# ArtyZe/yolo_quantization

Measured on AMD Instinct MI355X. Metric: images/sec yolov3-tiny INT8 416x416, higher is better.
Workload: dtype u8 x s8 -> int32 (f64 or exact-integer requant, bit-identical)

## Files before the change

yolo_quantization_amd/csrc/conv_rows.hip:

```cpp
#include "kargs.h"
#include <type_traits>

#if defined(MI355_ABLATE) && !defined(ROWS_TU_KS1)
#define DBG(bit) ((a.debug & (bit)) != 0)
#define TS_PHASES 6
#define TS_BLOCKS 4096
__device__ long long g_rows_ts[TS_PHASES][TS_BLOCKS];
#define TS(k)                                                                                   \
    do {                                                                                        \
        if (threadIdx.x == 0 && blockIdx.x < TS_BLOCKS) g_rows_ts[k][blockIdx.x] = wall_clock64(); \
    } while (0)
extern "C" int mi355_debug_read_ts(long long *host)
{
    return hipMemcpyFromSymbol(host, HIP_SYMBOL(g_rows_ts), sizeof(long long) * TS_PHASES * TS_BLOCKS) == hipSuccess ? 0 : -5;
}
#define WP_PHASES 5
__device__ long long g_rows_wp[TS_BLOCKS][8][WP_PHASES];
#define WP_DECL long long wp_acc[WP_PHASES] = {0, 0, 0, 0, 0}; long long wp_t = 0
#define WP_START()                                                   \
    do {                                                             \
        if (DBG(256)) { wp_t = __builtin_readcyclecounter(); }       \
    } while (0)
#define WP_MARK(k)                                                   \
    do {                                                             \
        if (DBG(256)) {                                              \
            asm volatile("s_waitcnt lgkmcnt(0)" ::: "memory");       \
            const long long wp_n = __builtin_readcyclecounter();     \
            wp_acc[k] += wp_n - wp_t;                                \
            wp_t = wp_n;                                             \
        }                                                            \
    } while (0)
#define WP_FLUSH()                                                                                   \
    do {                                                                                             \
        if (DBG(256) && lane == 0 && blockIdx.x < TS_BLOCKS && wave < 8)                             \
            for (int k = 0; k < WP_PHASES; ++k) g_rows_wp[blockIdx.x][wave][k] = wp_acc[k];          \
    } while (0)
extern "C" int mi355_debug_read_wp(long long *host)
{
    return hipMemcpyFromSymbol(host, HIP_SYMBOL(g_rows_wp), sizeof(long long) * TS_BLOCKS * 8 * WP_PHASES) == hipSuccess ? 0 : -5;
}
#else
#define DBG(bit) (false)
#define TS(k) do { } while (0)
#define WP_DECL do { } while (0)
#define WP_START() do { } while (0)
#define WP_MARK(k) do { } while (0)
#define WP_FLUSH() do { } while (0)
#endif

#define DMA16(gsrc, ldst)                                                                               \
    __builtin_amdgcn_global_load_lds((const __attribute__((address_space(1))) void *)(gsrc),           \
                                     (__attribute__((address_space(3))) void *)(ldst), 16, 0, 0)

template <int KS, int BN> constexpr int ra_stages() { return KS == 3 ? (BN <= 192 ? 4 : 6) : (BN <= 128 ? 4 : 3); }
template <int KS, int BN> constexpr int rb_stages() { return KS == 3 ? 2 : ra_stages<KS, BN>(); }
constexpr int rows_nb_slots(int BN, int RS, int NW, int KS)
{
    const int wmin = RS * 3 / 4, halo = KS == 3 ? 1 : 0;
    const int rows = (BN - 2 + wmin) / wmin + 1 + (BN - 2 + wmin * wmin) / (wmin * wmin) + 2 * halo;
    return (rows * (RS / 16) + NW - 1) / NW;
}

__device__ __forceinline__ void row_of_pixel(int n, int H, int W, FastDiv fd_hw, FastDiv fd_w, int &grow, int &x)
{
    const int hw = H * W;
    const int b = fd_div(n, fd_hw);
    const int r = n - b * hw;
    const int y = fd_div(r, fd_w);
    x = r - y * W;
    grow = b * (H + 1) + y + 1;
}

template <int BM, int BN, int WMW, int WNW, int RS, int KS>
__global__ __launch_bounds__(64 * WMW * WNW, 2) void conv_rows_i8_kernel(const ConvArgs a)
{
    constexpr int NW = WMW * WNW, NT = 64 * NW;
    constexpr int TM = BM / WMW, TN = BN / WNW;
    constexpr int MS = TM / 32, NS = TN / 32;
    constexpr int ACH = BM / 16;
    constexpr int DW = (NW == 8 && KS == 3) ? 4 : NW;
    constexpr int APT = (ACH + DW - 1) / DW;
    constexpr int HALO = (KS == 3) ? 1 : 0;
    constexpr int PIECEB = RS * 16;
    constexpr int CPR = RS / 16;
    constexpr int OSTR = BM + 4;
    constexpr int RA_STAGES = ra_stages<KS, BN>();
    constexpr int RB_STAGES = rb_stages<KS, BN>();
    constexpr int NBS = rows_nb_slots(BN, RS, DW, KS);
    constexpr int SPS = (NBS + 3) / 4;
    static_assert(TM % 32 == 0 && TN % 32 == 0, "wave tile must be a multiple of the 32x32 MFMA tile");

    extern __shared__ __attribute__((aligned(16))) char smem[];
    char *ldsA = smem;
    char *ldsB = smem + RA_STAGES * BM * 64;
    const int rowb = a.rowb;
    const int bbytes = a.rows_cap * rowb;
    int *ldsS = reinterpret_cast<int *>(ldsB + RB_STAGES * bbytes);
    double *ldsPM = reinterpret_cast<double *>(smem + a.lds_param_off);
    int *ldsPI = reinterpret_cast<int *>(ldsPM + 3 * BM);
    float *ldsYL = reinterpret_cast<float *>(ldsPI + 2 * BM);

    const int tid = threadIdx.x;
    const int lane = tid & 63;
    const int wave = __builtin_amdgcn_readfirstlane(tid >> 6);
    const int wm = wave / WNW, wn = wave % WNW;
    const int kh = lane >> 5, lj = lane & 31;
    const int dwave = wave & (DW - 1);
    const bool issuer = wave < DW;
    TS(0);

    int logical;
    {
        const int nb = gridDim.x, id = blockIdx.x;
        const int q = nb >> 3, r = nb & 7, xcd = id & 7, idx = id >> 3;
        logical = (xcd < r ? xcd * (q + 1) : r * (q + 1) + (xcd - r) * q) + idx;
    }
    int mtile, ntile;
    {
        const int blk = fd_div(logical, a.fd_ntper);
        const int rem = logical - blk * (a.xcd_mb * a.ntiles_n);
        ntile = fd_div(rem, a.fd_mb);
        mtile = blk * a.xcd_mb + (rem - ntile * a.xcd_mb);
    }
    const int n0 = ntile * a.tile_q + min(ntile, a.tile_r);
    const int n_end = n0 + a.tile_q + (ntile < a.tile_r ? 1 : 0);
    const int W1 = a.W + 1, hw = a.H * a.W;

    int gr0, x0;
    row_of_pixel(n0, a.H, a.W, a.fd_hw, a.fd_w, gr0, x0);
    int gr1, x1;
    row_of_pixel(n_end - 1, a.H, a.W, a.fd_hw, a.fd_w, gr1, x1);
    const int grow_first = gr0 - HALO;
    const int nrows = gr1 - gr0 + 1 + 2 * HALO;
    const int ndma = nrows * CPR;

    int bbase[NS];
    int prow[NS], pcol[NS];
    bool nvalid[NS];
#pragma unroll
    for (int ns = 0; ns < NS; ++ns) {
        const int n = n0 + (ns * WNW + wn) * 32 + lj;
        nvalid[ns] = n < n_end;
        int gr, x;
        row_of_pixel(nvalid[ns] ? n : n_end - 1, a.H, a.W, a.fd_hw, a.fd_w, gr, x);
        prow[ns] = gr - grow_first - HALO;
        pcol[ns] = x + 1 - HALO;
        bbase[ns] = prow[ns] * rowb + pcol[ns] * 16 + kh * PIECEB;
    }
    int atab[MS];
#pragma unroll
    for (int ms = 0; ms < MS; ++ms) {
        const int row = wm * TM + ms * 32 + lj;
        atab[ms] = ((row >> 4) << 10) + ((row & 15) << 4) + kh * 256;
    }

    const unsigned lds0 = (unsigned)(size_t)(__attribute__((address_space(3))) char *)smem;
#define DMA_S(ldsdst_u32, sbase_ptr, voff_u32)                                                                   \
    asm volatile("s_mov_b32 m0, %0\n\ts_nop 0\n\tglobal_load_lds_dwordx4 %1, %2" ::"s"(ldsdst_u32), "v"(voff_u32), \
                 "s"(sbase_ptr)                                                                                  \
                 : "memory", "m0")
    constexpr int TAPS = KS * KS;
    const int rot = a.debug & 512 ? 0 : ntile - fd_div(ntile, a.fd_nch) * a.nchunks;
    const int kwrap = a.ksteps;
    int aleft = kwrap - rot * TAPS;
    const int8_t *aptr[APT];
    unsigned adst[APT];
#pragma unroll
    for (int i = 0; i < APT; ++i) {
        const int ch = min(dwave + i * DW, ACH - 1);
        aptr[i] = a.wp + ((size_t)(mtile * ACH + ch) * a.ksteps + (size_t)rot * TAPS) * 1024;
        adst[i] = lds0 + (ch << 10);
    }
    const unsigned lane16 = lane * 16;
// ... 210 lines not shown
                        for (int ms = 0; ms < MS; ++ms) rot[st][ms] = aaddr[(st + ROT) % R][ms];
#pragma unroll
                    for (int st = 0; st < R; ++st)
#pragma unroll
                        for (int ms = 0; ms < MS; ++ms) aaddr[st][ms] = rot[st][ms];
#pragma unroll
                    for (int yy = 0; yy < 3; ++yy)
#pragma unroll
                        for (int ns = 0; ns < NS; ++ns) baddr[yy][ns] += bdelta;
                }
                WP_MARK(0);
                if (t > 0 || chunk > 0) {
                    asm volatile("s_waitcnt vmcnt(%0)" ::"n"(YOUNG) : "memory");
                    WP_MARK(1);
                    if (!DBG(2)) __builtin_amdgcn_s_barrier();
                    WP_MARK(2);
                }
                half(fa[C0], fb[C0], fa[N0], fb[N0], aaddr[SN], baddr[TYN], integral_constant<int, TAPN>{},
                     integral_constant<int, 0>{}, integral_constant<bool, RD>{}, true_type{}, [&] {
                         if (!LAST && t < 4 && !DBG(1))
                             issueB_slots(chunk + 1, integral_constant<int, BLO>{}, integral_constant<int, BHI>{});
                         if (ISSUE_A && !DBG(1)) {
                             if constexpr (R == 6) {
                                 constexpr unsigned E = ((t + R - 1) % R) * (BM * 64), O = ((t + R - 1 + 3) % R) * (BM * 64);
                                 issueA_next(odd ? O : E);
                             } else {
                                 issueA_next((unsigned)((chunk + t + R - 1) & 3) * (BM * 64));
                             }
                         }
                     });
                WP_MARK(3);
                half(fa[C1], fb[C1], fa[N1], fb[N1], aaddr[SN], baddr[TYN], integral_constant<int, TAPN>{},
                     integral_constant<int, 1>{}, integral_constant<bool, RD>{}, integral_constant<bool, RD>{}, nohook);
                WP_MARK(4);
                if (t == 1 && !DBG(16)) {
                    asm volatile("s_waitcnt lgkmcnt(0)" ::: "memory");
                    cell_sums(Bt);
                    asm volatile("s_waitcnt lgkmcnt(0)" ::: "memory");
                    __builtin_amdgcn_sched_barrier(0);
                }
            };
            step(integral_constant<int, 0>{}); step(integral_constant<int, 1>{}); step(integral_constant<int, 2>{});
            step(integral_constant<int, 3>{}); step(integral_constant<int, 4>{}); step(integral_constant<int, 5>{});
            step(integral_constant<int, 6>{}); step(integral_constant<int, 7>{}); step(integral_constant<int, 8>{});
        };
        for (int chunk = 0; chunk + 1 < a.nchunks; ++chunk) chunk_body(false_type{}, chunk);
        chunk_body(true_type{}, a.nchunks - 1);
        asm volatile("s_waitcnt lgkmcnt(0)" ::: "memory");
        WP_FLUSH();
#undef LDS_READ128
    } else {
        TS(2);
        constexpr int R1 = RA_STAGES;
        constexpr int G = NBS + APT;
        static_assert(RB_STAGES == R1 && (R1 == 3 || R1 == 4), "1x1 loop: common ring depth");
        for (int g0 = 0; g0 < a.ksteps; g0 += R1) {
#pragma unroll
            for (int u = 0; u < R1; ++u) {
                const int g = g0 + u;
                if (g < a.ksteps) {
                    const int young = min(R1 - 2, a.ksteps - 1 - g);
                    if (young == R1 - 2) asm volatile("s_waitcnt vmcnt(%0)" ::"n"((R1 - 2) * G) : "memory");
                    else if (young == 1) asm volatile("s_waitcnt vmcnt(%0)" ::"n"(G) : "memory");
                    else asm volatile("s_waitcnt vmcnt(0)" ::: "memory");
                    __builtin_amdgcn_s_barrier();
                    if (g + R1 - 1 < a.ksteps) {
                        issueB(g + R1 - 1);
                        issueA_next(((u + R1 - 1) % R1) * (BM * 64));
                    }
                    const char *Bt = ldsB + u * bbytes;
                    compute(ldsA + u * (BM * 64), Bt, 0);
                    __builtin_amdgcn_sched_barrier(0);
                }
            }
        }
    }

    TS(3);
    if (DBG(32)) {
        if (acc[0][0][0] == 0x7fffffff && a.y) a.y[tid] = 1;
        return;
    }
    __syncthreads();
    int sx[NS];
#pragma unroll
    for (int ns = 0; ns < NS; ++ns) {
        int t = 0;
        if (KS == 1) {
            t = sxr[ns] + __shfl_xor(sxr[ns], 32);
        } else {
            const int c0 = prow[ns] * RS + pcol[ns];
#pragma unroll
            for (int dy = 0; dy < KS; ++dy)
#pragma unroll
                for (int dx = 0; dx < KS; ++dx) t += ldsS[c0 + dy * RS + dx];
        }
        sx[ns] = t;
    }
    __syncthreads();
    char *otile = smem;
    int *celltab = reinterpret_cast<int *>(smem + BN * OSTR);
    const int m0 = mtile * BM;

    int pb_[NS], rem[NS], nl_[NS];
#pragma unroll
    for (int ns = 0; ns < NS; ++ns) {
        const int nl = (ns * WNW + wn) * 32 + lj;
        nl_[ns] = nl;
        const int nn = nvalid[ns] ? n0 + nl : 0;
        const int b = fd_div(nn, a.fd_hw);
        const int rem0 = nn - b * hw;
        const int y = fd_div(rem0, a.fd_w), xx = rem0 - y * a.W;
        pb_[ns] = b;
        rem[ns] = rem0;
        if (wm == 0 && kh == 0) {
            const int up = a.up;
            celltab[nl] = !nvalid[ns] ? -1
                          : up == 1   ? a.out_lead + (b * (a.H + 1) + (y + 1)) * W1 + xx
                                      : a.out_lead + (b * (up * a.H + 1) + (up * y + 1)) * (up * a.W + 1) + up * xx;
        }
    }
    const bool fast = !a.acc_out && a.hdr->pow2 == 1;
    auto epi_fast = [&](auto act_c, auto sat_c) {
        constexpr int ACT = decltype(act_c)::value;
        constexpr bool SAT = decltype(sat_c)::value != 0;
#pragma unroll
        for (int ms = 0; ms < MS; ++ms) {
#pragma unroll
            for (int grp = 0; grp < 4; ++grp) {
                const int ocl = wm * TM + ms * 32 + 8 * grp + 4 * kh;
                const int4 dz4 = *reinterpret_cast<const int4 *>(ldsPI + ocl);
                const int dzv[4] = {dz4.x, dz4.y, dz4.z, dz4.w};
                int32_t accb[4][NS];
                double mp[4];
#pragma unroll
                for (int r = 0; r < 4; ++r) {
                    mp[r] = ldsPM[2 * BM + ocl + r];
#pragma unroll
                    for (int ns = 0; ns < NS; ++ns)
                        accb[r][ns] = acc[ms][ns][grp * 4 + r] + __mul24(dzv[r], sx[ns]);
                }
                int32_t v[4][NS];
                requant_values<ACT, SAT, NS>(accb, mp, a.zp_act, v);
#pragma unroll
                for (int ns = 0; ns < NS; ++ns)
                    *reinterpret_cast<uint32_t *>(otile + nl_[ns] * OSTR + ocl) = pack4_biased(v[0][ns], v[1][ns], v[2][ns], v[3][ns]);
                if (a.y_f32) {
#pragma unroll
                    for (int r = 0; r < 4; ++r) {
                        const int oc = m0 + ocl + r;
                        if (oc < a.n) {
                            const int e = a.yolo_out ? oc % a.yolo_per : 0;
#pragma unroll
                            for (int ns = 0; ns < NS; ++ns)
                                if (nvalid[ns]) {
                                    const int u8 = v[r][ns] & 0xFF;
                                    const float f = (float)(u8 - a.zp_act) * a.s_act;
                                    const size_t ridx = ((size_t)pb_[ns] * a.n + oc) * hw + rem[ns];
                                    a.y_f32[ridx] = f;
                                    if (a.yolo_out) a.yolo_out[ridx] = (e == 2 || e == 3) ? f : ldsYL[u8];
                                }
                        }
                    }
                }
            }
        }
    };
    using std::integral_constant;
    if (DBG(64)) {
    } else if (fast) {
#ifdef MI355_EPI_ONE
        epi_fast(integral_constant<int, MI355_ACT_LEAKY>{}, integral_constant<int, 0>{});
    }
    if (false) {
#endif
        const bool sat = a.store_mode == MI355_STORE_SATURATE;
        if (a.act == MI355_ACT_LEAKY) {
            if (sat) epi_fast(integral_constant<int, MI355_ACT_LEAKY>{}, integral_constant<int, 1>{});
            else epi_fast(integral_constant<int, MI355_ACT_LEAKY>{}, integral_constant<int, 0>{});
        } else if (a.act == MI355_ACT_RELU6) {
            if (sat) epi_fast(integral_constant<int, MI355_ACT_RELU6>{}, integral_constant<int, 1>{});
            else epi_fast(integral_constant<int, MI355_ACT_RELU6>{}, integral_constant<int, 0>{});
        } else {
            if (sat) epi_fast(integral_constant<int, MI355_ACT_LINEAR>{}, integral_constant<int, 1>{});
            else epi_fast(integral_constant<int, MI355_ACT_LINEAR>{}, integral_constant<int, 0>{});
        }
    }
#ifndef MI355_EPI_ONE
    else {
    #pragma unroll
        for (int ms = 0; ms < MS; ++ms) {
    #pragma unroll
            for (int grp = 0; grp < 4; ++grp) {
                const int ocl = wm * TM + ms * 32 + 8 * grp + 4 * kh;
                const int oc0 = m0 + ocl;
                if (oc0 >= a.n) {
    #pragma unroll
                    for (int ns = 0; ns < NS; ++ns) *reinterpret_cast<uint32_t *>(otile + nl_[ns] * OSTR + ocl) = 0x80808080u;
                    continue;
                }
                uint32_t packed[NS];
    #pragma unroll
                for (int ns = 0; ns < NS; ++ns) packed[ns] = 0;
    #pragma unroll
                for (int r = 0; r < 4; ++r) {
                    const int oc = oc0 + r;
                    const int dzv = ldsPI[ocl + r], biv = ldsPI[BM + ocl + r];
                    const double mv = ldsPM[ocl + r], sv = ldsPM[BM + ocl + r];
    #pragma unroll
                    for (int ns = 0; ns < NS; ++ns) {
                        const int32_t accv = acc[ms][ns][grp * 4 + r] - biv + dzv * sx[ns];
                        uint32_t u8 = 0;
                        if (oc < a.n) {
                            u8 = requant_u8(accv, biv, mv, sv, a.zp_act, a.act, a.store_mode);
                            if (nvalid[ns] && (a.acc_out || a.y_f32)) {
                                const size_t ridx = ((size_t)pb_[ns] * a.n + oc) * hw + rem[ns];
                                if (a.acc_out) a.acc_out[ridx] = accv;
                                if (a.y_f32) {
                                    const float f = (float)((int)u8 - a.zp_act) * a.s_act;
                                    a.y_f32[ridx] = f;
                                    if (a.yolo_out) {
                                        const int e = oc % a.yolo_per;
                                        a.yolo_out[ridx] = (e == 2 || e == 3) ? f : ldsYL[u8];
                                    }
                                }
                            }
                        }
                        packed[ns] |= (u8 ^ 0x80u) << (8 * r);
                    }
                }
    #pragma unroll
                for (int ns = 0; ns < NS; ++ns) *reinterpret_cast<uint32_t *>(otile + nl_[ns] * OSTR + ocl) = packed[ns];
            }
        }
    }
#endif
    __syncthreads();
    TS(4);
    if (a.y && !DBG(128)) {
        const int dwords = min(BM, a.out_w - m0) >> 2;
        if (a.up > 1) {
            const int total = BN * dwords, rowc = a.up * a.W + 1;
            for (int p = tid; p < total; p += NT) {
                const int pix = p / dwords, d = p - pix * dwords;
                const int cell = celltab[pix];
                if (cell >= 0) {
                    const uint32_t v = *reinterpret_cast<const uint32_t *>(otile + pix * OSTR + d * 4);
                    for (int uy = 0; uy < a.up; ++uy)
                        for (int ux = 0; ux < a.up; ++ux)
                            *reinterpret_cast<uint32_t *>(a.y + (size_t)(cell + uy * rowc + ux) * a.out_cs + m0 + d * 4) = v;
                }
            }
        } else if (dwords == BM / 4 && !(a.out_cs & 15) && !((size_t)a.y & 15)) {
#pragma unroll 2
            for (int p = tid; p < BN * (BM / 16); p += NT) {
                const int pix = p / (BM / 16), q = p % (BM / 16);
                const int cell = celltab[pix];
                if (cell >= 0) {
                    const uint32_t *sp = reinterpret_cast<const uint32_t *>(otile + pix * OSTR + q * 16);
                    const uint4 v = make_uint4(sp[0], sp[1], sp[2], sp[3]);
                    *reinterpret_cast<uint4 *>(a.y + (size_t)cell * a.out_cs + m0 + q * 16) = v;
                }
            }
        } else if (dwords == BM / 4) {
#pragma unroll 4
            for (int p = tid; p < BN * (BM / 4); p += NT) {
                const int pix = p / (BM / 4), d = p % (BM / 4);
                const int cell = celltab[pix];
                if (cell >= 0)
                    *reinterpret_cast<uint32_t *>(a.y + (size_t)cell * a.out_cs + m0 + d * 4) =
                        *reinterpret_cast<const uint32_t *>(otile + pix * OSTR + d * 4);
            }
        } else {
            const int total = BN * dwords;
            for (int p = tid; p < total; p += NT) {
                const int pix = p / dwords, d = p - pix * dwords;
                const int cell = celltab[pix];
                if (cell >= 0)
                    *reinterpret_cast<uint32_t *>(a.y + (size_t)cell * a.out_cs + m0 + d * 4) =
                        *reinterpret_cast<const uint32_t *>(otile + pix * OSTR + d * 4);
            }
        }
    }
    TS(5);
}

template <int BM, int BN, int WMW, int WNW, int RS, int KS>
static int rows_launch_cfg(ConvArgs &a, hipStream_t st)
{
    constexpr int NW = WMW * WNW, NT = 64 * NW;
    constexpr int DW = (NW == 8 && KS == 3) ? 4 : NW;
    constexpr int HALO = (KS == 3) ? 1 : 0;
    if (a.mpad % BM) return MI355_EINVAL;
    a.mtiles = a.mpad / BM;
    if (a.ntiles_n < (a.total_n + BN - 1) / BN) a.ntiles_n = (a.total_n + BN - 1) / BN;
    a.rows_cap = (BN - 2 + a.W) / a.W + 1 + (BN - 2 + a.H * a.W) / (a.H * a.W) + 2 * HALO;
    const int ndma = a.rows_cap * (RS / 16);
    if ((ndma + DW - 1) / DW > rows_nb_slots(BN, RS, DW, KS)) return MI355_EINVAL;
    if ((size_t)a.in_cells * (size_t)a.in_cs >= ((size_t)1 << 32)) return MI355_EINVAL;
    a.rowb = RS * 64 + 16 * (a.W & 15);
    a.fd_hw = fastdiv_make((uint32_t)(a.H * a.W)); a.fd_w = fastdiv_make((uint32_t)a.W);
    a.fd_ntn = fastdiv_make((uint32_t)a.ntiles_n); a.fd_nch = fastdiv_make((uint32_t)a.nchunks);
    a.tile_q = a.total_n / a.ntiles_n; a.tile_r = a.total_n % a.ntiles_n;
    size_t lds = (size_t)ra_stages<KS, BN>() * BM * 64 + (size_t)rb_stages<KS, BN>() * a.rows_cap * a.rowb + (size_t)a.rows_cap * RS * 4;
    const size_t lds_epi = (size_t)BN * (BM + 4) + (size_t)BN * 4;
    if (lds_epi > lds) lds = lds_epi;
    lds = (lds + 15) & ~(size_t)15;
    a.lds_param_off = (int)lds;
    lds += (size_t)BM * 32 + (a.yolo_out ? 1024 : 0);
    if (lds > 160 * 1024) return MI355_EINVAL;
    auto kern = conv_rows_i8_kernel<BM, BN, WMW, WNW, RS, KS>;
    static size_t lds_attr_dev[64] = {0};
    int dev_ix = 0;
    (void)hipGetDevice(&dev_ix);
    size_t &lds_attr = lds_attr_dev[dev_ix & 63];
    if (lds > 64 * 1024 && lds > lds_attr) {
        lds_attr = lds;
        if (hipFuncSetAttribute(reinterpret_cast<const void *>(kern), hipFuncAttributeMaxDynamicSharedMemorySize,
                                (int)lds) != hipSuccess)
            return MI355_EHIP;
    }
    a.xcd_mb = 1;
    if (!(a.debug & (1 << 24))) {
        const long nb = (long)a.ntiles_n * a.mtiles, per = (nb + 7) / 8;
        const double wslab = (double)BM * a.ksteps * 64, itile = (double)a.total_n / a.ntiles_n * a.cb * a.nchunks;
        double best = 0;
        for (int mb = 1; mb <= a.mtiles; ++mb) {
            if (a.mtiles % mb) continue;
            const long blk = (long)mb * a.ntiles_n;
            const long mt = std::min<long>(a.mtiles, mb * ((per + blk - 1) / blk)), nt = std::min<long>(a.ntiles_n, (per + mb - 1) / mb + (per % mb || blk % per || nb % 8 ? 1 : 0));
            const double bytes = mt * wslab + nt * itile;
            if (mb == 1 || bytes < best) { best = bytes; a.xcd_mb = mb; }
        }
    }
    a.fd_ntper = fastdiv_make((uint32_t)(a.xcd_mb * a.ntiles_n));
    a.fd_mb = fastdiv_make((uint32_t)a.xcd_mb);
    dim3 grid(a.ntiles_n * a.mtiles), block(NT);
    conv_launch_note(grid.x, NT, lds);
    hipLaunchKernelGGL(kern, grid, block, lds, st, a);
    return hipGetLastError() == hipSuccess ? MI355_OK : MI355_EHIP;
}

template <int RS, int KS>
static int rows_launch_tile(ConvArgs &a, hipStream_t st, int bm, int bn)
{
    if (bm == 128 && bn == 384) return rows_launch_cfg<128, 384, 2, 4, RS, KS>(a, st);
    if (bm == 128 && bn == 256) return rows_launch_cfg<128, 256, 2, 4, RS, KS>(a, st);
    if constexpr (KS == 3) {
        if (bm == 128 && bn == 192) return rows_launch_cfg<128, 192, 2, 2, RS, KS>(a, st);
    }
    if (bm == 128 && bn == 128) return rows_launch_cfg<128, 128, 2, 2, RS, KS>(a, st);
    if (bm == 64 && bn == 256) return rows_launch_cfg<64, 256, 1, 4, RS, KS>(a, st);
    if (bm == 64 && bn == 128) return rows_launch_cfg<64, 128, 1, 4, RS, KS>(a, st);
    if (bm == 32 && bn == 256) return rows_launch_cfg<32, 256, 1, 4, RS, KS>(a, st);
    if (bm == 32 && bn == 128) return rows_launch_cfg<32, 128, 1, 4, RS, KS>(a, st);
    return MI355_EINVAL;
}

// ... 30 lines not shown
```

yolo_quantization_amd/csrc/conv_rows16.hip:

```cpp
#include "kargs.h"
#include <type_traits>

#if defined(MI355_ABLATE)
#define DBG(bit) ((a.debug & (bit)) != 0)
__device__ long long g_rows16_ts[6][4096];
#define TS(k) do { if (threadIdx.x == 0 && blockIdx.x < 4096) g_rows16_ts[k][blockIdx.x] = wall_clock64(); } while (0)
extern "C" int mi355_debug_read_ts16(long long *host)
{
    return hipMemcpyFromSymbol(host, HIP_SYMBOL(g_rows16_ts), sizeof(long long) * 6 * 4096) == hipSuccess ? 0 : -5;
}
#else
#define DBG(bit) (false)
#define TS(k) do { } while (0)
#endif
#define WP_DECL do { } while (0)
#define WP_START() do { } while (0)
#define WP_MARK(k) do { } while (0)
#define WP_FLUSH() do { } while (0)

#define DMA16(gsrc, ldst)                                                                               \
    __builtin_amdgcn_global_load_lds((const __attribute__((address_space(1))) void *)(gsrc),           \
                                     (__attribute__((address_space(3))) void *)(ldst), 16, 0, 0)

template <int KS, int BN> constexpr int ra16_stages() { return KS == 3 ? (BN <= 192 ? 4 : 6) : (BN <= 128 ? 4 : 3); }
template <int KS, int BN> constexpr int rb16_stages() { return KS == 3 ? 2 : ra16_stages<KS, BN>(); }
constexpr int rows16_nb_slots(int BN, int RS, int NW, int KS)
{
    const int wmin = RS * 3 / 4, halo = KS == 3 ? 1 : 0;
    const int rows = (BN - 2 + wmin) / wmin + 1 + (BN - 2 + wmin * wmin) / (wmin * wmin) + 2 * halo;
    return (rows * (RS / 16) + NW - 1) / NW;
}

__device__ __forceinline__ void row16_of_pixel(int n, int H, int W, FastDiv fd_hw, FastDiv fd_w, int &grow, int &x)
{
    const int hw = H * W;
    const int b = fd_div(n, fd_hw);
    const int r = n - b * hw;
    const int y = fd_div(r, fd_w);
    x = r - y * W;
    grow = b * (H + 1) + y + 1;
}

template <int BM, int BN, int WMW, int WNW, int RS, int KS, int NBX = 0>
__global__ __launch_bounds__(64 * WMW * WNW, (BM / WMW > 64 ? 1 : 2)) void conv_rows16_i8_kernel(const ConvArgs a)
{
    constexpr int NW = WMW * WNW, NT = 64 * NW;
    constexpr int TM = BM / WMW, TN = BN / WNW;
    constexpr int MI = TM / 16, NI = TN / 16;
    constexpr int ACH = BM / 16;
    static_assert(KS == 3 && TN % 32 == 0, "3x3 only; pixels are dealt in 32-column sub-tiles (two 16-column tiles each)");
    constexpr int DW = (NW == 8 && KS == 3) ? 4 : NW;
    constexpr int APT = (ACH + DW - 1) / DW;
    constexpr int HALO = (KS == 3) ? 1 : 0;
    constexpr int PIECEB = RS * 16;
    constexpr int CPR = RS / 16;
    constexpr int OSTR = BM + 4;
    constexpr int RA_STAGES = ra16_stages<KS, BN>();
    constexpr int RB_STAGES = rb16_stages<KS, BN>();
    constexpr int NBS = rows16_nb_slots(BN, RS, DW, KS) + NBX;
    constexpr int SPS = (NBS + 3) / 4;
    static_assert(TM % 16 == 0 && TN % 32 == 0, "wave tile: 16-row tiles, 32-column sub-tiles");
    constexpr int CPT = (NBS * DW * 16 + NT - 1) / NT;
    static_assert(CPT * NT >= NBS * DW * 16 && CPT >= 1 && CPT <= 2, "a chunk's 4 CPT piece reads ride on its K-steps 0..7, one each");
    constexpr bool COUNTED = CPT == 1;
    constexpr auto cs_slot = [](int t) { return !COUNTED ? -1 : CPT == 2 ? (t >= 0 && t < 8 ? t : -1) : (t >= 0 && t < 8 && !(t & 1) ? t >> 1 : -1); };

    extern __shared__ __attribute__((aligned(16))) char smem[];
    char *ldsB = smem + RA_STAGES * BM * 64;
    const int rowb = a.rowb;
    const int bbytes = a.rows_cap * rowb;
    int *ldsS = reinterpret_cast<int *>(ldsB + RB_STAGES * bbytes);
    double *ldsPM = reinterpret_cast<double *>(smem + a.lds_param_off);
    int *ldsPI = reinterpret_cast<int *>(ldsPM + 3 * BM);
    float *ldsYL = reinterpret_cast<float *>(ldsPI + 2 * BM);

    const int tid = threadIdx.x;
    const int lane = tid & 63;
    const int wave = __builtin_amdgcn_readfirstlane(tid >> 6);
    const int wm = wave / WNW, wn = wave % WNW;
    const int kq = lane >> 4, lj = lane & 15;
    const int dwave = wave & (DW - 1);
    const bool issuer = wave < DW;
    TS(0);

    int logical;
    {
        const int nb = gridDim.x, id = blockIdx.x;
        const int q = nb >> 3, r = nb & 7, xcd = id & 7, idx = id >> 3;
        logical = (xcd < r ? xcd * (q + 1) : r * (q + 1) + (xcd - r) * q) + idx;
    }
    int mtile, ntile;
    {
        const int blk = fd_div(logical, a.fd_ntper);
        const int rem = logical - blk * (a.xcd_mb * a.ntiles_n);
        ntile = fd_div(rem, a.fd_mb);
        mtile = blk * a.xcd_mb + (rem - ntile * a.xcd_mb);
    }
    const int n0 = ntile * a.tile_q + min(ntile, a.tile_r);
    const int n_end = n0 + a.tile_q + (ntile < a.tile_r ? 1 : 0);
    const int W1 = a.W + 1, hw = a.H * a.W;

    int gr0, x0;
    row16_of_pixel(n0, a.H, a.W, a.fd_hw, a.fd_w, gr0, x0);
    int gr1, x1;
    row16_of_pixel(n_end - 1, a.H, a.W, a.fd_hw, a.fd_w, gr1, x1);
    const int grow_first = gr0 - HALO;
    const int nrows = gr1 - gr0 + 1 + 2 * HALO;
    const int ndma = nrows * CPR;

    constexpr int NS = NI;
    int bbase[NS];
#pragma unroll
    for (int ns = 0; ns < NS; ++ns) {
        const int n = n0 + ((ns >> 1) * WNW + wn) * 32 + (ns & 1) * 16 + lj;
        int gr, x;
        row16_of_pixel(n < n_end ? n : n_end - 1, a.H, a.W, a.fd_hw, a.fd_w, gr, x);
        const int prow = gr - grow_first - HALO;
        const int pcol = x + 1 - HALO;
        bbase[ns] = prow * rowb + pcol * 16 + kq * PIECEB;
    }
    const int atab0 = (wm * MI) * 1024 + lane * 16;

    const unsigned lds0 = (unsigned)(size_t)(__attribute__((address_space(3))) char *)smem;
#define DMA_S(ldsdst_u32, sbase_ptr, voff_u32)                                                                   \
    asm volatile("s_mov_b32 m0, %0\n\ts_nop 0\n\tglobal_load_lds_dwordx4 %1, %2" ::"s"(ldsdst_u32), "v"(voff_u32), \
                 "s"(sbase_ptr)                                                                                  \
                 : "memory", "m0")
    constexpr int TAPS = KS * KS;
    const int rot = a.debug & 512 ? 0 : ntile - fd_div(ntile, a.fd_nch) * a.nchunks;
    const int kwrap = a.ksteps;
    int aleft = kwrap - rot * TAPS;
    const int8_t *aptr[APT];
    unsigned adst[APT];
#pragma unroll
    for (int i = 0; i < APT; ++i) {
        const int ch = min(dwave + i * DW, ACH - 1);
        aptr[i] = a.wp + ((size_t)(mtile * ACH + ch) * a.ksteps + (size_t)rot * TAPS) * 1024;
        adst[i] = lds0 + (ch << 10);
    }
    const unsigned lane16 = lane * 16;
    auto issueA_next = [&](unsigned stage_off) {
        if (DW < NW && !issuer) return;
// ... 180 lines not shown
                if (t == 2 || t == 5) {
#pragma unroll
                    for (int ni = 0; ni < NI; ++ni) baddr[ni] += rowb;
                }
                if (t > 0 || chunk > 0) {
                    asm volatile("s_waitcnt vmcnt(%0)" ::"n"(YOUNG) : "memory");
                    __builtin_amdgcn_s_barrier();
                }
                auto dma = [&] {
                    __builtin_amdgcn_sched_barrier(0);
                    if (!LAST && t < 4) issueB_slots(chunk + 1, integral_constant<int, BLO>{}, integral_constant<int, BHI>{});
                    if (ISSUE_A) {
                        if constexpr (R == 6) {
                            constexpr unsigned E = ((t + R - 1) % R) * (BM * 64), O = ((t + R - 1 + 3) % R) * (BM * 64);
                            issueA_next(odd ? O : E);
                        } else if constexpr (R == 5) {
                            issueA_next(sst[t == 8 ? (t + R - 1 - 9) % R : (t + R - 1) % R]);
                        } else {
                            issueA_next((unsigned)((chunk + t + R - 1) & 3) * (BM * 64));
                        }
                    }
                    __builtin_amdgcn_sched_barrier(0);
                };
                asm volatile("s_waitcnt lgkmcnt(2)" ::: "memory");
                __builtin_amdgcn_sched_barrier(0);
#pragma unroll
                for (int ni = 0; ni < NI - 2; ++ni) {
#pragma unroll
                    for (int mi = 0; mi < MI; ++mi) {
                        acc[mi][ni] = __builtin_amdgcn_mfma_i32_16x16x64_i8(fa[mi], fb[ni], acc[mi][ni], 0, 0, 0);
                        if (ni == 0 && mi == 0) dma();
                    }
                    __builtin_amdgcn_sched_barrier(0);
                    if (RD) LDS_READ128(fb[ni], baddr[ni], TAPN);
                    __builtin_amdgcn_sched_barrier(0);
                    if (ni == 0) cell_piece();
                }
                if (RD) asm volatile("s_waitcnt lgkmcnt(%0)" ::"n"(NI - 2 + (NI > 2 && CJ >= 0 ? 1 : 0)) : "memory");
                else asm volatile("s_waitcnt lgkmcnt(0)" ::: "memory");
                __builtin_amdgcn_sched_barrier(0);
#pragma unroll
                for (int mi = 0; mi < MI; ++mi) {
                    acc[mi][NI - 2] = __builtin_amdgcn_mfma_i32_16x16x64_i8(fa[mi], fb[NI - 2], acc[mi][NI - 2], 0, 0, 0);
                    if (NI == 2 && mi == 0) dma();
                    acc[mi][NI - 1] = __builtin_amdgcn_mfma_i32_16x16x64_i8(fa[mi], fb[NI - 1], acc[mi][NI - 1], 0, 0, 0);
                    __builtin_amdgcn_sched_barrier(0);
                    if (RD) LDS_READ128(fa[mi], aaddr[SN], mi * 1024);
                    __builtin_amdgcn_sched_barrier(0);
                    if (NI == 2 && mi == 0) cell_piece();
                }
                if (RD) {
                    LDS_READ128(fb[NI - 2], baddr[NI - 2], TAPN);
                    LDS_READ128(fb[NI - 1], baddr[NI - 1], TAPN);
                }
                __builtin_amdgcn_sched_barrier(0);
                if (!COUNTED && t == 1 && !DBG(16)) {
                    asm volatile("s_waitcnt lgkmcnt(0)" ::: "memory");
                    cell_sums(Bt);
                    asm volatile("s_waitcnt lgkmcnt(0)" ::: "memory");
                    __builtin_amdgcn_sched_barrier(0);
                }
            };
            step(integral_constant<int, 0>{}); step(integral_constant<int, 1>{}); step(integral_constant<int, 2>{});
            step(integral_constant<int, 3>{}); step(integral_constant<int, 4>{}); step(integral_constant<int, 5>{});
            step(integral_constant<int, 6>{}); step(integral_constant<int, 7>{}); step(integral_constant<int, 8>{});
        };
        for (int chunk = 0; chunk + 1 < a.nchunks; ++chunk) chunk_body(false_type{}, chunk);
        chunk_body(true_type{}, a.nchunks - 1);
        asm volatile("s_waitcnt lgkmcnt(0)" ::: "memory");
        if constexpr (COUNTED) {
#pragma unroll
            for (int k = 0; k < CPT; ++k)
                if (tid + k * NT < nrows * RS) ldsS[tid + k * NT] = csum[k];
        }
#undef LDS_READ128
    }

    TS(3);
    if (DBG(32)) {
        if (acc[0][0][0] == 0x7fffffff && a.y) a.y[tid] = 1;
        return;
    }
    __syncthreads();
    int sx[NS];
    bool nvalid[NS];
#pragma unroll
    for (int ns = 0; ns < NS; ++ns) {
        int t = 0;
        const int n = n0 + ((ns >> 1) * WNW + wn) * 32 + (ns & 1) * 16 + lj;
        nvalid[ns] = n < n_end;
        int gr, x;
        row16_of_pixel(nvalid[ns] ? n : n_end - 1, a.H, a.W, a.fd_hw, a.fd_w, gr, x);
        const int c0 = (gr - grow_first - HALO) * RS + x + 1 - HALO;
#pragma unroll
        for (int dy = 0; dy < KS; ++dy)
#pragma unroll
            for (int dx = 0; dx < KS; ++dx) t += ldsS[c0 + dy * RS + dx];
        sx[ns] = t;
    }
    __syncthreads();
    char *otile = smem;
    int *celltab = reinterpret_cast<int *>(smem + BN * OSTR);
    const int m0 = mtile * BM;

    int pb_[NS], rem[NS], nl_[NS];
#pragma unroll
    for (int ns = 0; ns < NS; ++ns) {
        const int nl = ((ns >> 1) * WNW + wn) * 32 + (ns & 1) * 16 + lj;
        nl_[ns] = nl;
        const int nn = nvalid[ns] ? n0 + nl : 0;
        const int b = fd_div(nn, a.fd_hw);
        const int rem0 = nn - b * hw;
        const int y = fd_div(rem0, a.fd_w), xx = rem0 - y * a.W;
        pb_[ns] = b;
        rem[ns] = rem0;
        if (wm == 0 && kq == 0) {
            const int up = a.up;
            celltab[nl] = !nvalid[ns] ? -1
                          : up == 1   ? a.out_lead + (b * (a.H + 1) + (y + 1)) * W1 + xx
                                      : a.out_lead + (b * (up * a.H + 1) + (up * y + 1)) * (up * a.W + 1) + up * xx;
        }
    }
    const bool fast = !a.acc_out && a.hdr->pow2 == 1;
    auto epi_fast = [&](auto act_c, auto sat_c) {
        constexpr int ACT = decltype(act_c)::value;
        constexpr bool SAT = decltype(sat_c)::value != 0;
        constexpr int NH = (NS % 3 == 0) ? 3 : 2;
        static_assert(NS % NH == 0, "pixel tiles per lane");
#pragma unroll
        for (int mi = 0; mi < MI; ++mi) {
            const int ocl = wm * TM + mi * 16 + 4 * kq;
            const int4 dz4 = *reinterpret_cast<const int4 *>(ldsPI + ocl);
            const int dzv[4] = {dz4.x, dz4.y, dz4.z, dz4.w};
            double mp[4];
#pragma unroll
            for (int r = 0; r < 4; ++r) mp[r] = ldsPM[2 * BM + ocl + r];
#pragma unroll
            for (int n0h = 0; n0h < NS; n0h += NH) {
                int32_t accb[4][NH];
#pragma unroll
                for (int r = 0; r < 4; ++r)
#pragma unroll
                    for (int k = 0; k < NH; ++k)
                        accb[r][k] = acc[mi][n0h + k][r] + __mul24(dzv[r], sx[n0h + k]);
                int32_t v[4][NH];
                requant_values<ACT, SAT, NH>(accb, mp, a.zp_act, v);
#pragma unroll
                for (int k = 0; k < NH; ++k)
                    *reinterpret_cast<uint32_t *>(otile + nl_[n0h + k] * OSTR + ocl) = pack4_biased(v[0][k], v[1][k], v[2][k], v[3][k]);
                if (a.y_f32) {
#pragma unroll
                    for (int r = 0; r < 4; ++r) {
                        const int oc = m0 + ocl + r;
                        if (oc < a.n) {
                            const int e = a.yolo_out ? oc % a.yolo_per : 0;
#pragma unroll
                            for (int k = 0; k < NH; ++k)
                                if (nvalid[n0h + k]) {
                                    const int u8 = v[r][k] & 0xFF;
                                    const float f = (float)(u8 - a.zp_act) * a.s_act;
                                    const size_t ridx = ((size_t)pb_[n0h + k] * a.n + oc) * hw + rem[n0h + k];
                                    a.y_f32[ridx] = f;
                                    if (a.yolo_out) a.yolo_out[ridx] = (e == 2 || e == 3) ? f : ldsYL[u8];
                                }
                        }
                    }
                }
            }
        }
    };
    using std::integral_constant;
    if (DBG(64)) {
    } else if (fast) {
#ifdef MI355_EPI_ONE
        epi_fast(integral_constant<int, MI355_ACT_LEAKY>{}, integral_constant<int, 0>{});
    }
    if (false) {
#endif
        const bool sat = a.store_mode == MI355_STORE_SATURATE;
        if (a.act == MI355_ACT_LEAKY) {
            if (sat) epi_fast(integral_constant<int, MI355_ACT_LEAKY>{}, integral_constant<int, 1>{});
            else epi_fast(integral_constant<int, MI355_ACT_LEAKY>{}, integral_constant<int, 0>{});
        } else if (a.act == MI355_ACT_RELU6) {
            if (sat) epi_fast(integral_constant<int, MI355_ACT_RELU6>{}, integral_constant<int, 1>{});
            else epi_fast(integral_constant<int, MI355_ACT_RELU6>{}, integral_constant<int, 0>{});
        } else {
            if (sat) epi_fast(integral_constant<int, MI355_ACT_LINEAR>{}, integral_constant<int, 1>{});
            else epi_fast(integral_constant<int, MI355_ACT_LINEAR>{}, integral_constant<int, 0>{});
        }
    }
#ifndef MI355_EPI_ONE
    else {
#pragma unroll
        for (int mi = 0; mi < MI; ++mi) {
            const int ocl = wm * TM + mi * 16 + 4 * kq;
            const int oc0 = m0 + ocl;
            if (oc0 >= a.n) {
#pragma unroll
                for (int ns = 0; ns < NS; ++ns) *reinterpret_cast<uint32_t *>(otile + nl_[ns] * OSTR + ocl) = 0x80808080u;
                continue;
            }
            uint32_t packed[NS];
#pragma unroll
            for (int ns = 0; ns < NS; ++ns) packed[ns] = 0;
#pragma unroll
            for (int r = 0; r < 4; ++r) {
                const int oc = oc0 + r;
                const int dzv = ldsPI[ocl + r], biv = ldsPI[BM + ocl + r];
                const double mv = ldsPM[ocl + r], sv = ldsPM[BM + ocl + r];
#pragma unroll
                for (int ns = 0; ns < NS; ++ns) {
                    const int32_t accv = acc[mi][ns][r] - biv + dzv * sx[ns];
                    uint32_t u8 = 0;
                    if (oc < a.n) {
                        u8 = requant_u8(accv, biv, mv, sv, a.zp_act, a.act, a.store_mode);
                        if (nvalid[ns] && (a.acc_out || a.y_f32)) {
                            const size_t ridx = ((size_t)pb_[ns] * a.n + oc) * hw + rem[ns];
                            if (a.acc_out) a.acc_out[ridx] = accv;
                            if (a.y_f32) {
                                const float f = (float)((int)u8 - a.zp_act) * a.s_act;
                                a.y_f32[ridx] = f;
                                if (a.yolo_out) {
                                    const int e = oc % a.yolo_per;
                                    a.yolo_out[ridx] = (e == 2 || e == 3) ? f : ldsYL[u8];
                                }
                            }
                        }
                    }
                    packed[ns] |= (u8 ^ 0x80u) << (8 * r);
                }
            }
#pragma unroll
            for (int ns = 0; ns < NS; ++ns) *reinterpret_cast<uint32_t *>(otile + nl_[ns] * OSTR + ocl) = packed[ns];
        }
    }
#endif
    __syncthreads();
    TS(4);
    if (a.y && !DBG(128)) {
        const int dwords = min(BM, a.out_w - m0) >> 2;
        if (a.up > 1) {
            const int total = BN * dwords, rowc = a.up * a.W + 1;
            for (int p = tid; p < total; p += NT) {
                const int pix = p / dwords, d = p - pix * dwords;
                const int cell = celltab[pix];
                if (cell >= 0) {
                    const uint32_t v = *reinterpret_cast<const uint32_t *>(otile + pix * OSTR + d * 4);
                    for (int uy = 0; uy < a.up; ++uy)
                        for (int ux = 0; ux < a.up; ++ux)
                            *reinterpret_cast<uint32_t *>(a.y + (size_t)(cell + uy * rowc + ux) * a.out_cs + m0 + d * 4) = v;
                }
            }
        } else if (dwords == BM / 4 && !(a.out_cs & 15) && !((size_t)a.y & 15)) {
#pragma unroll 2
            for (int p = tid; p < BN * (BM / 16); p += NT) {
                const int pix = p / (BM / 16), q = p % (BM / 16);
                const int cell = celltab[pix];
                if (cell >= 0) {
                    const uint32_t *sp = reinterpret_cast<const uint32_t *>(otile + pix * OSTR + q * 16);
                    const uint4 v = make_uint4(sp[0], sp[1], sp[2], sp[3]);
                    *reinterpret_cast<uint4 *>(a.y + (size_t)cell * a.out_cs + m0 + q * 16) = v;
                }
            }
        } else if (dwords == BM / 4) {
#pragma unroll 4
            for (int p = tid; p < BN * (BM / 4); p += NT) {
                const int pix = p / (BM / 4), d = p % (BM / 4);
                const int cell = celltab[pix];
                if (cell >= 0)
                    *reinterpret_cast<uint32_t *>(a.y + (size_t)cell * a.out_cs + m0 + d * 4) =
                        *reinterpret_cast<const uint32_t *>(otile + pix * OSTR + d * 4);
            }
        } else {
            const int total = BN * dwords;
            for (int p = tid; p < total; p += NT) {
                const int pix = p / dwords, d = p - pix * dwords;
                const int cell = celltab[pix];
                if (cell >= 0)
                    *reinterpret_cast<uint32_t *>(a.y + (size_t)cell * a.out_cs + m0 + d * 4) =
                        *reinterpret_cast<const uint32_t *>(otile + pix * OSTR + d * 4);
            }
        }
    }
    TS(5);
}

template <int BM, int BN, int WMW, int WNW, int RS, int KS, int NBX = 0>
static int rows16_launch_cfg(ConvArgs &a, hipStream_t st)
{
    constexpr int NW = WMW * WNW, NT = 64 * NW;
    constexpr int DW = (NW == 8 && KS == 3) ? 4 : NW;
    constexpr int HALO = (KS == 3) ? 1 : 0;
    if (a.mpad % BM) return MI355_EINVAL;
    a.mtiles = a.mpad / BM;
    if (a.ntiles_n < (a.total_n + BN - 1) / BN) a.ntiles_n = (a.total_n + BN - 1) / BN;
    a.tile_q = a.total_n / a.ntiles_n; a.tile_r = a.total_n % a.ntiles_n;
    {
        const int hw = a.H * a.W;
        auto grow = [&](long n) { const long b = n / hw, r = n - b * hw; return (int)(b * (a.H + 1) + r / a.W + 1); };
        int span = 0;
        for (int t = 0; t < a.ntiles_n; ++t) {
            const long n0 = (long)t * a.tile_q + (t < a.tile_r ? t : a.tile_r), n1 = n0 + a.tile_q + (t < a.tile_r ? 1 : 0) - 1;
            if (n1 < n0) continue;
            const int sp = grow(n1) - grow(n0) + 1;
            if (sp > span) span = sp;
        }
        a.rows_cap = span + 2 * HALO;
    }
    const int ndma = a.rows_cap * (RS / 16);
    if ((ndma + DW - 1) / DW > rows16_nb_slots(BN, RS, DW, KS) + NBX) return MI355_EINVAL;
    if ((size_t)a.in_cells * (size_t)a.in_cs >= ((size_t)1 << 32)) return MI355_EINVAL;
    a.rowb = RS * 64 + 16 * (a.W & 15);
    a.fd_hw = fastdiv_make((uint32_t)(a.H * a.W)); a.fd_w = fastdiv_make((uint32_t)a.W);
    a.fd_ntn = fastdiv_make((uint32_t)a.ntiles_n); a.fd_nch = fastdiv_make((uint32_t)a.nchunks);
    size_t lds = (size_t)ra16_stages<KS, BN>() * BM * 64 + (size_t)rb16_stages<KS, BN>() * a.rows_cap * a.rowb + (size_t)a.rows_cap * RS * 4;
    const size_t lds_epi = (size_t)BN * (BM + 4) + (size_t)BN * 4;
    if (lds_epi > lds) lds = lds_epi;
    lds = (lds + 15) & ~(size_t)15;
    a.lds_param_off = (int)lds;
    lds += (size_t)BM * 32 + (a.yolo_out ? 1024 : 0);
    if (lds > 160 * 1024) return MI355_EINVAL;
    auto kern = conv_rows16_i8_kernel<BM, BN, WMW, WNW, RS, KS, NBX>;
// ... 52 lines not shown
```

Measured before the change: 277,600.

## Store conv epilogue outputs directly from registers via permlane swaps, skipping LDS tile

For the 128x128 tile configs of both the 32-row and 16-row conv kernels, the epilogue now rearranges the packed output bytes across lanes with permlane16/32 swaps. Each lane then writes 16-byte vectors straight to global memory instead of staging the tile in LDS. This removes the LDS write, two block barriers and the cooperative readback loop when the fast path applies (no upsample, aligned output, full channel tile). The trade is less coalesced per-lane global stores and added shuffle instructions. An asm barrier on tid is added to keep lane-index math in VGPRs.

```diff
diff --git a/yolo_quantization_amd/csrc/conv_rows.hip b/yolo_quantization_amd/csrc/conv_rows.hip
--- a/yolo_quantization_amd/csrc/conv_rows.hip
+++ b/yolo_quantization_amd/csrc/conv_rows.hip
@@ -89,6 +89,11 @@
     constexpr int NBS = rows_nb_slots(BN, RS, DW, KS);
     constexpr int SPS = (NBS + 3) / 4;
     static_assert(TM % 32 == 0 && TN % 32 == 0, "wave tile must be a multiple of the 32x32 MFMA tile");
+#ifdef MI355_ROWS_LDS_TILE
+    constexpr bool REGST = false;
+#else
+    constexpr bool REGST = KS == 3 && BM == 128 && BN == 128;
+#endif
 
     extern __shared__ __attribute__((aligned(16))) char smem[];
     char *ldsA = smem;
@@ -465,6 +470,12 @@
         return;
     }
     __syncthreads();
+    int tid_e = tid;
+    asm volatile("" : "+v"(tid_e));
+    const int kh_e = (tid_e >> 5) & 1, lj_e = tid_e & 31;
+    bool nvalid_e[NS];
+#pragma unroll
+    for (int ns = 0; ns < NS; ++ns) nvalid_e[ns] = n0 + (ns * WNW + wn) * 32 + lj_e < n_end;
     int sx[NS];
 #pragma unroll
     for (int ns = 0; ns < NS; ++ns) {
@@ -480,38 +491,44 @@
         }
         sx[ns] = t;
     }
-    __syncthreads();
+    const int m0 = mtile * BM;
+    const bool fast = !a.acc_out && a.hdr->pow2 == 1;
+    const bool regst = REGST && fast && a.y && a.up == 1 && a.out_w - m0 >= BM && !(a.out_cs & 15) && !((size_t)a.y & 15) && !(a.debug & 32768);
+    const bool lds_tile = !regst && !DBG(262144);
+    if (lds_tile) __syncthreads();
     char *otile = smem;
     int *celltab = reinterpret_cast<int *>(smem + BN * OSTR);
-    const int m0 = mtile * BM;
 
     int pb_[NS], rem[NS], nl_[NS];
+    int stcell[NS] = {};
 #pragma unroll
     for (int ns = 0; ns < NS; ++ns) {
-        const int nl = (ns * WNW + wn) * 32 + lj;
+        const int nl = (ns * WNW + wn) * 32 + lj_e;
         nl_[ns] = nl;
-        const int nn = nvalid[ns] ? n0 + nl : 0;
+        const int nn = nvalid_e[ns] ? n0 + nl : 0;
         const int b = fd_div(nn, a.fd_hw);
         const int rem0 = nn - b * hw;
         const int y = fd_div(rem0, a.fd_w), xx = rem0 - y * a.W;
         pb_[ns] = b;
         rem[ns] = rem0;
-        if (wm == 0 && kh == 0) {
+        if (REGST && regst) {
+            stcell[ns] = a.out_lead + (b * (a.H + 1) + (y + 1)) * W1 + xx;
+        } else if (wm == 0 && kh_e == 0 && lds_tile) {
             const int up = a.up;
-            celltab[nl] = !nvalid[ns] ? -1
+            celltab[nl] = !nvalid_e[ns] ? -1
                           : up == 1   ? a.out_lead + (b * (a.H + 1) + (y + 1)) * W1 + xx
                                       : a.out_lead + (b * (up * a.H + 1) + (up * y + 1)) * (up * a.W + 1) + up * xx;
         }
     }
-    const bool fast = !a.acc_out && a.hdr->pow2 == 1;
     auto epi_fast = [&](auto act_c, auto sat_c) {
         constexpr int ACT = decltype(act_c)::value;
         constexpr bool SAT = decltype(sat_c)::value != 0;
 #pragma unroll
         for (int ms = 0; ms < MS; ++ms) {
+            uint32_t pk[4][NS];
 #pragma unroll
             for (int grp = 0; grp < 4; ++grp) {
-                const int ocl = wm * TM + ms * 32 + 8 * grp + 4 * kh;
+                const int ocl = wm * TM + ms * 32 + 8 * grp + 4 * kh_e;
                 const int4 dz4 = *reinterpret_cast<const int4 *>(ldsPI + ocl);
                 const int dzv[4] = {dz4.x, dz4.y, dz4.z, dz4.w};
                 int32_t accb[4][NS];
@@ -526,8 +543,11 @@
                 int32_t v[4][NS];
                 requant_values<ACT, SAT, NS>(accb, mp, a.zp_act, v);
 #pragma unroll
-                for (int ns = 0; ns < NS; ++ns)
-                    *reinterpret_cast<uint32_t *>(otile + nl_[ns] * OSTR + ocl) = pack4_biased(v[0][ns], v[1][ns], v[2][ns], v[3][ns]);
+                for (int ns = 0; ns < NS; ++ns) {
+                    pk[grp][ns] = pack4_biased(v[0][ns], v[1][ns], v[2][ns], v[3][ns]);
+                    if (DBG(262144)) asm volatile("" ::"v"(pk[grp][ns]));
+                    else if (!REGST || !regst) *reinterpret_cast<uint32_t *>(otile + nl_[ns] * OSTR + ocl) = pk[grp][ns];
+                }
                 if (a.y_f32) {
 #pragma unroll
                     for (int r = 0; r < 4; ++r) {
@@ -536,7 +556,7 @@
                             const int e = a.yolo_out ? oc % a.yolo_per : 0;
 #pragma unroll
                             for (int ns = 0; ns < NS; ++ns)
-                                if (nvalid[ns]) {
+                                if (nvalid_e[ns]) {
                                     const int u8 = v[r][ns] & 0xFF;
                                     const float f = (float)(u8 - a.zp_act) * a.s_act;
                                     const size_t ridx = ((size_t)pb_[ns] * a.n + oc) * hw + rem[ns];
@@ -544,6 +564,18 @@
                                     if (a.yolo_out) a.yolo_out[ridx] = (e == 2 || e == 3) ? f : ldsYL[u8];
                                 }
                         }
+                    }
+                }
+            }
+            if constexpr (REGST) {
+                if (regst) {
+#pragma unroll
+                    for (int ns = 0; ns < NS; ++ns) {
+                        const auto s02 = __builtin_amdgcn_permlane32_swap(pk[0][ns], pk[2][ns], false, false);
+                        const auto s13 = __builtin_amdgcn_permlane32_swap(pk[1][ns], pk[3][ns], false, false);
+                        const uint4 dq = make_uint4(s02[0], s02[1], s13[0], s13[1]);
+                        if (DBG(128)) asm volatile("" ::"v"(dq.x), "v"(dq.y), "v"(dq.z), "v"(dq.w));
+                        else if (nvalid_e[ns]) *reinterpret_cast<uint4 *>(a.y + (size_t)stcell[ns] * a.out_cs + (m0 + wm * TM + ms * 32 + 16 * kh_e)) = dq;
                     }
                 }
             }
@@ -575,7 +607,7 @@
         for (int ms = 0; ms < MS; ++ms) {
     #pragma unroll
             for (int grp = 0; grp < 4; ++grp) {
-                const int ocl = wm * TM + ms * 32 + 8 * grp + 4 * kh;
+                const int ocl = wm * TM + ms * 32 + 8 * grp + 4 * kh_e;
                 const int oc0 = m0 + ocl;
                 if (oc0 >= a.n) {
     #pragma unroll
@@ -596,7 +628,7 @@
                         uint32_t u8 = 0;
                         if (oc < a.n) {
                             u8 = requant_u8(accv, biv, mv, sv, a.zp_act, a.act, a.store_mode);
-                            if (nvalid[ns] && (a.acc_out || a.y_f32)) {
+                            if (nvalid_e[ns] && (a.acc_out || a.y_f32)) {
                                 const size_t ridx = ((size_t)pb_[ns] * a.n + oc) * hw + rem[ns];
                                 if (a.acc_out) a.acc_out[ridx] = accv;
                                 if (a.y_f32) {
@@ -618,13 +650,13 @@
         }
     }
 #endif
-    __syncthreads();
+    if (lds_tile) __syncthreads();
     TS(4);
-    if (a.y && !DBG(128)) {
+    if (lds_tile && a.y && !DBG(128)) {
         const int dwords = min(BM, a.out_w - m0) >> 2;
         if (a.up > 1) {
             const int total = BN * dwords, rowc = a.up * a.W + 1;
-            for (int p = tid; p < total; p += NT) {
+            for (int p = tid_e; p < total; p += NT) {
                 const int pix = p / dwords, d = p - pix * dwords;
                 const int cell = celltab[pix];
                 if (cell >= 0) {
@@ -636,7 +668,7 @@
             }
         } else if (dwords == BM / 4 && !(a.out_cs & 15) && !((size_t)a.y & 15)) {
 #pragma unroll 2
-            for (int p = tid; p < BN * (BM / 16); p += NT) {
+            for (int p = tid_e; p < BN * (BM / 16); p += NT) {
                 const int pix = p / (BM / 16), q = p % (BM / 16);
                 const int cell = celltab[pix];
                 if (cell >= 0) {
@@ -647,7 +679,7 @@
             }
         } else if (dwords == BM / 4) {
 #pragma unroll 4
-            for (int p = tid; p < BN * (BM / 4); p += NT) {
+            for (int p = tid_e; p < BN * (BM / 4); p += NT) {
                 const int pix = p / (BM / 4), d = p % (BM / 4);
                 const int cell = celltab[pix];
                 if (cell >= 0)
@@ -656,7 +688,7 @@
             }
         } else {
             const int total = BN * dwords;
-            for (int p = tid; p < total; p += NT) {
+            for (int p = tid_e; p < total; p += NT) {
                 const int pix = p / dwords, d = p - pix * dwords;
                 const int cell = celltab[pix];
                 if (cell >= 0)
diff --git a/yolo_quantization_amd/csrc/conv_rows16.hip b/yolo_quantization_amd/csrc/conv_rows16.hip
--- a/yolo_quantization_amd/csrc/conv_rows16.hip
+++ b/yolo_quantization_amd/csrc/conv_rows16.hip
@@ -58,6 +58,11 @@
     constexpr int RA_STAGES = ra16_stages<KS, BN>();
     constexpr int RB_STAGES = rb16_stages<KS, BN>();
     constexpr int NBS = rows16_nb_slots(BN, RS, DW, KS) + NBX;
+#ifdef MI355_ROWS_LDS_TILE
+    constexpr bool REGST = false;
+#else
+    constexpr bool REGST = TN / 16 == 4 && BM == 128 && BN == 128;
+#endif
     constexpr int SPS = (NBS + 3) / 4;
     static_assert(TM % 16 == 0 && TN % 32 == 0, "wave tile: 16-row tiles, 32-column sub-tiles");
     constexpr int CPT = (NBS * DW * 16 + NT - 1) / NT;
@@ -404,46 +409,56 @@
         return;
     }
     __syncthreads();
+    const int m0 = mtile * BM;
+    const bool fast = !a.acc_out && a.hdr->pow2 == 1;
+    const bool regst = REGST && fast && a.y && a.up == 1 && a.out_w - m0 >= BM && !(a.out_cs & 15) && !((size_t)a.y & 15) && !(a.debug & 32768);
     int sx[NS];
     bool nvalid[NS];
+    int pb_[NS], rem[NS], nl_[NS];
+    int stcell = 0;
+    bool stvalid = false;
 #pragma unroll
     for (int ns = 0; ns < NS; ++ns) {
         int t = 0;
-        const int n = n0 + ((ns >> 1) * WNW + wn) * 32 + (ns & 1) * 16 + lj;
+        const int nl = ((ns >> 1) * WNW + wn) * 32 + (ns & 1) * 16 + lj;
+        const int n = n0 + nl;
+        nl_[ns] = nl;
         nvalid[ns] = n < n_end;
-        int gr, x;
-        row16_of_pixel(nvalid[ns] ? n : n_end - 1, a.H, a.W, a.fd_hw, a.fd_w, gr, x);
+        const int nn = nvalid[ns] ? n : n_end - 1;
+        const int b = fd_div(nn, a.fd_hw);
+        const int rem0 = nn - b * hw;
+        const int y = fd_div(rem0, a.fd_w), x = rem0 - y * a.W;
+        const int gr = b * (a.H + 1) + y + 1;
         const int c0 = (gr - grow_first - HALO) * RS + x + 1 - HALO;
 #pragma unroll
         for (int dy = 0; dy < KS; ++dy)
 #pragma unroll
             for (int dx = 0; dx < KS; ++dx) t += ldsS[c0 + dy * RS + dx];
         sx[ns] = t;
-    }
-    __syncthreads();
+        pb_[ns] = b;
+        rem[ns] = rem0;
+        if (REGST && kq == ns) {
+            stcell = a.out_lead + gr * W1 + x;
+            stvalid = nvalid[ns];
+        }
+    }
     char *otile = smem;
     int *celltab = reinterpret_cast<int *>(smem + BN * OSTR);
-    const int m0 = mtile * BM;
-
-    int pb_[NS], rem[NS], nl_[NS];
-#pragma unroll
-    for (int ns = 0; ns < NS; ++ns) {
-        const int nl = ((ns >> 1) * WNW + wn) * 32 + (ns & 1) * 16 + lj;
-        nl_[ns] = nl;
-        const int nn = nvalid[ns] ? n0 + nl : 0;
-        const int b = fd_div(nn, a.fd_hw);
-        const int rem0 = nn - b * hw;
-        const int y = fd_div(rem0, a.fd_w), xx = rem0 - y * a.W;
-        pb_[ns] = b;
-        rem[ns] = rem0;
+    const bool lds_tile = !regst && !DBG(262144);
+    if (lds_tile) {
+        __syncthreads();
         if (wm == 0 && kq == 0) {
-            const int up = a.up;
-            celltab[nl] = !nvalid[ns] ? -1
-                          : up == 1   ? a.out_lead + (b * (a.H + 1) + (y + 1)) * W1 + xx
-                                      : a.out_lead + (b * (up * a.H + 1) + (up * y + 1)) * (up * a.W + 1) + up * xx;
-        }
-    }
-    const bool fast = !a.acc_out && a.hdr->pow2 == 1;
+#pragma unroll
+            for (int ns = 0; ns < NS; ++ns) {
+                const int up = a.up, b = pb_[ns];
+                const int y = fd_div(rem[ns], a.fd_w), xx = rem[ns] - y * a.W;
+                celltab[nl_[ns]] = !nvalid[ns] ? -1
+                                   : up == 1   ? a.out_lead + (b * (a.H + 1) + (y + 1)) * W1 + xx
+                                               : a.out_lead + (b * (up * a.H + 1) + (up * y + 1)) * (up * a.W + 1) + up * xx;
+            }
+        }
+    }
+    char *const stp = reinterpret_cast<char *>(a.y) + (size_t)stcell * a.out_cs + m0 + wm * TM;
     auto epi_fast = [&](auto act_c, auto sat_c) {
         constexpr int ACT = decltype(act_c)::value;
         constexpr bool SAT = decltype(sat_c)::value != 0;
@@ -457,6 +472,7 @@
             double mp[4];
 #pragma unroll
             for (int r = 0; r < 4; ++r) mp[r] = ldsPM[2 * BM + ocl + r];
+            uint32_t pk[NS];
 #pragma unroll
             for (int n0h = 0; n0h < NS; n0h += NH) {
                 int32_t accb[4][NH];
@@ -468,8 +484,11 @@
                 int32_t v[4][NH];
                 requant_values<ACT, SAT, NH>(accb, mp, a.zp_act, v);
 #pragma unroll
-                for (int k = 0; k < NH; ++k)
-                    *reinterpret_cast<uint32_t *>(otile + nl_[n0h + k] * OSTR + ocl) = pack4_biased(v[0][k], v[1][k], v[2][k], v[3][k]);
+                for (int k = 0; k < NH; ++k) {
+                    pk[n0h + k] = pack4_biased(v[0][k], v[1][k], v[2][k], v[3][k]);
+                    if (DBG(262144)) asm volatile("" ::"v"(pk[n0h + k]));
+                    else if (!REGST || !regst) *reinterpret_cast<uint32_t *>(otile + nl_[n0h + k] * OSTR + ocl) = pk[n0h + k];
+                }
                 if (a.y_f32) {
 #pragma unroll
                     for (int r = 0; r < 4; ++r) {
@@ -487,6 +506,17 @@
                                 }
                         }
                     }
+                }
+            }
+            if constexpr (REGST) {
+                if (regst) {
+                    const auto p01 = __builtin_amdgcn_permlane16_swap(pk[0], pk[1], false, false);
+                    const auto p23 = __builtin_amdgcn_permlane16_swap(pk[2], pk[3], false, false);
+                    const auto q02 = __builtin_amdgcn_permlane32_swap(p01[0], p23[0], false, false);
+                    const auto q13 = __builtin_amdgcn_permlane32_swap(p01[1], p23[1], false, false);
+                    const uint4 dq = make_uint4(q02[0], q13[0], q02[1], q13[1]);
+                    if (DBG(128)) asm volatile("" ::"v"(dq.x), "v"(dq.y), "v"(dq.z), "v"(dq.w));
+                    else if (stvalid) *reinterpret_cast<uint4 *>(stp + mi * 16) = dq;
                 }
             }
         }
@@ -557,9 +587,9 @@
         }
     }
 #endif
-    __syncthreads();
+    if (lds_tile) __syncthreads();
     TS(4);
-    if (a.y && !DBG(128)) {
+    if (lds_tile && a.y && !DBG(128)) {
         const int dwords = min(BM, a.out_w - m0) >> 2;
         if (a.up > 1) {
             const int total = BN * dwords, rowc = a.up * a.W + 1;
```

New measurement: 272,300. 0.981x the previous value.
